# apcamargo/genomad

Hardware: NVIDIA H100
Metric: nn_classification_windows_per_s (higher is better)
Workload: dtype split operands on wgmma (conv: fp16 main pass + two e4m3 correction passes; w_v: 3 fp16 passes), fp32 accumulate; fp32-equivalent (<=1e-4 vs the fp32 oracle, measured ~1e-5)

## Files before the change

### genomad_b200/csrc/api.cu

```cuda
#include <cuda.h>
#include <cuda_runtime.h>
#include <cuda_fp16.h>

#include <algorithm>
#include <cmath>
#include <cstdio>
#include <cstring>
#include <string>
#include <vector>

#include <cub/device/device_radix_sort.cuh>
#include <cub/device/device_scan.cuh>

#include "../../include/gnm.h"
#include "common.cuh"
#include "encode.cuh"
#include "conv_t.cuh"
#include "layer1_wv.cuh"
#include "conv_ref.cuh"
#include "igloo.cuh"
#include "dense.cuh"
#include "logits_tc.cuh"
#include "wv_gather.cuh"
#include "contigs.cuh"
// ... 295 lines not shown
                                float* ent_w, int32_t* groups, int* n_groups, int32_t* band_first_group, uint32_t* frag, float* unscale,
                                int* layout) {
  if (layout) { layout[0] = kBandRows; layout[1] = kNumBands; layout[2] = kGsSlots; layout[3] = kWgGroupMax; }
  if (!patches && !w_mult && !w_summer) return 0;
  if (!patches || !w_mult || !w_summer || !n_groups) return fail("gnm_pack_patches: null argument");
  for (int i = 0; i < kPatches * kPatchLen; ++i)
    if (patches[i] < 0 || patches[i] >= kTok) return fail("gnm_pack_patches: patch index out of range");
  PatchPack pk;
  if (!pack_patches(patches, w_mult, w_summer, pk))
    return fail("gnm_pack_patches: folded patch weights w_mult * w_summer / 32 not finite: no fp16 operand split carries them");
  const int real_groups = pk.band_gstart[kNumBands];
  if (groups && *n_groups < real_groups) return fail("gnm_pack_patches: groups buffer too small");
  if (slot_of) std::memcpy(slot_of, pk.slot_of.data(), pk.slot_of.size() * sizeof(int32_t));
  if (ent_pos) std::memcpy(ent_pos, pk.ent_pos.data(), pk.ent_pos.size() * sizeof(int32_t));
  if (ent_w) std::memcpy(ent_w, pk.ent_w.data(), pk.ent_w.size() * sizeof(float));
  if (groups) for (int i = 0; i < real_groups; ++i) { groups[2 * i] = pk.groups[i].x; groups[2 * i + 1] = pk.groups[i].y; }
  *n_groups = real_groups;
  if (band_first_group) std::memcpy(band_first_group, pk.band_gstart.data(), pk.band_gstart.size() * sizeof(int32_t));
  if (frag) std::memcpy(frag, pk.frag.data(), pk.frag.size() * sizeof(uint32_t));
  if (unscale) *unscale = pk.unscale;
  return 0;
}

static void fold_bn(const gnm_bn_weights& b, std::vector<float>& sc, std::vector<float>& sh) {
  sc.resize(kHidden); sh.resize(kHidden);
  for (int i = 0; i < kHidden; ++i) {
    const float inv = b.gamma[i] * (1.0f / std::sqrt(b.moving_variance[i] + 1e-3f));
    sc[i] = inv;
    sh[i] = b.beta[i] - b.moving_mean[i] * inv;
  }
}

static void split_dense_t(const float* w, int K, std::vector<float>& thi, std::vector<float>& tlo) {
  thi.resize(static_cast<size_t>(kHidden) * K); tlo.resize(thi.size());
  for (int k = 0; k < K; ++k)
    for (int n = 0; n < kHidden; ++n)
      split_tf32(w[static_cast<size_t>(k) * kHidden + n], thi[static_cast<size_t>(n) * K + k], tlo[static_cast<size_t>(n) * K + k]);
}

extern "C" int gnm_create(int device, const gnm_weights* w, int max_batch, gnm_handle** out) {
  if (!w || !out) return fail("gnm_create: null argument");
  if (max_batch < 1 || max_batch > 32768) return fail("gnm_create: max_batch must be in [1, 32768]");
  int ndev = 0;
  if (cudaGetDeviceCount(&ndev) != cudaSuccess || ndev == 0)
    return fail("gnm_create: no CUDA device available (libgnm has no CPU fallback)");
  if (device < 0 || device >= ndev) return fail("gnm_create: bad device index");
// ... 2529 lines not shown
```

### genomad_b200/csrc/conv_t.cuh

```cuda
#pragma once
#include <cuda.h>
#include "common.cuh"

namespace gnm {

constexpr int kTileM       = 128;
constexpr int kUnitsPerWin = (kTok + 2 * kTileM - 1) / (2 * kTileM);
constexpr int kSlabRows    = 136;
constexpr int kARegion     = kSlabRows * 128;
constexpr int kA2Region    = 2 * kARegion;
constexpr int kNumRegions  = 4;
constexpr int kA2Bytes     = kNumRegions * kA2Region;
constexpr int kBStage      = 128 * 128;
constexpr int kBHalf       = kBStage / 2;
constexpr int kConvThreads = 384;
constexpr int kConvStages  = 24;
constexpr int kWvStages    = 4;
constexpr int kTWSlots     = 5;
constexpr int kEpiTile     = 512;
constexpr int kEpiStage    = 8 * 2 * kEpiTile;
constexpr int kConvTSmem   = kA2Bytes + 2 * kTWSlots * kBHalf + kEpiStage + 2048;
static_assert(kConvTSmem <= 232448, "conv_t_kernel exceeds the 227 KB of shared memory a CTA may use");

struct ConvTcParams {
  const float* bias;
  uint8_t* y_out;
  float* q_out;
  float out_scale;
  int out_fp8;
  int n_tiles;
  int experiment;
  long long* dbg;
  DeviceStatus* status;
};

template <bool kWvMode> __device__ __forceinline__ int conv_pack_stage(int q) {
  return kWvMode ? q : ((q / 6 + 2) & 3) * 6 + q % 6;
}
template <bool kWvMode> __device__ __forceinline__ constexpr int region_src(int r) {
  return kWvMode ? (r == 0 ? kOffHi16 : r == 1 ? kOffHi16 + 128 : r == 2 ? kOffLo16 : kOffLo16 + 128)
                 : (r == 0 ? kOffHi16 : r == 1 ? kOffHi16 + 128 : r == 2 ? kOffP8 : kOffP8 + 128);
}

constexpr int kConvFwd = 0, kConvWv = 1, kConvRoute = 2, kConvBwd = 3;
struct ConvAttrExt {
  uint8_t* route_out;
  const uint8_t* mask_rows;
  const float* add_rows;
  const float* s_w;
  const float* s_in;
  float* f32_out;
  float* unit_max;
};

template <int kMode>
__device__ __forceinline__ void conv_t_body(const CUtensorMap* tm_act_p, const CUtensorMap* tm_w_p, const ConvTcParams& p,
                                            const ConvAttrExt& x) {
  constexpr bool kWvMode = kMode == kConvWv || kMode == kConvRoute;
  constexpr int kStagesU = kWvMode ? kWvStages : kConvStages;
  extern __shared__ uint8_t smem_raw[];
  uint8_t* smem = reinterpret_cast<uint8_t*>((reinterpret_cast<uintptr_t>(smem_raw) + 1023) & ~uintptr_t(1023));
  uint8_t* s_a = smem;
  uint8_t* s_w = smem + kA2Bytes;
  uint8_t* s_epi = s_w + 2 * kTWSlots * kBHalf;
  uint64_t* bars = reinterpret_cast<uint64_t*>(s_epi + kEpiStage);
  uint64_t* a_full = bars;
  uint64_t* a_empty = bars + 4;
  uint64_t* w_full = bars + 8;
  uint64_t* w_empty = bars + 8 + 2 * kTWSlots;

  const int warp = __shfl_sync(0xffffffffu, static_cast<int>(threadIdx.x) >> 5, 0);
  const int wg = warp >> 2, wq = warp & 3, lane = threadIdx.x & 31;
  const int n_units = p.n_tiles;

  if (threadIdx.x == 0) {
    tma_prefetch_desc(tm_act_p);
    tma_prefetch_desc(tm_w_p);
    for (int i = 0; i < kNumRegions; ++i) { mbar_init(&a_full[i], 1); mbar_init(&a_empty[i], 8); }
    for (int i = 0; i < 2 * kTWSlots; ++i) { mbar_init(&w_full[i], 1); mbar_init(&w_empty[i], 4); }
    fence_barrier_init();
  }
  __syncthreads();

  if (wg == 0) {
    if (wq == 0 && elect_one()) {
      uint32_t wcount = 0;
      const uint64_t pol = l2_policy_evict_last();
      for (int unit = blockIdx.x; unit < n_units; unit += gridDim.x, wcount += kStagesU)
        for (int g = 0; g < 2; ++g)
          for (int q = 0; q < kStagesU; ++q) {
            const int s = g * kTWSlots + (wcount + q) % kTWSlots;
            const uint32_t wphase = ((wcount + q) / kTWSlots) & 1;
            mbar_wait(&w_empty[s], wphase ^ 1, p.status, 110 + s);
            mbar_arrive_expect_tx(&w_full[s], kBHalf);
            tma_load_2d_hint(s_w + s * kBHalf, tm_w_p, &w_full[s], 0, conv_pack_stage<kWvMode>(q) * 128 + 64 * g, pol);
          }
    } else if (wq == 1 && elect_one()) {
      int it = 0;
      const uint64_t pol = l2_policy_evict_first();
      for (int unit = blockIdx.x; unit < n_units; unit += gridDim.x, ++it) {
        const uint32_t ph = it & 1;
        const int w = unit / kUnitsPerWin;
        const int t0 = (unit - w * kUnitsPerWin) * (2 * kTileM);
#pragma unroll
        for (int k = 0; k < kNumRegions; ++k) {
          const int r = kWvMode ? (k == 0 ? 0 : k == 1 ? 2 : k == 2 ? 1 : 3) : (k + 2) & 3;
          mbar_wait(&a_empty[r], ph ^ 1, p.status, 100 + r);
          mbar_arrive_expect_tx(&a_full[r], kA2Region);
          uint8_t* dst = s_a + r * kA2Region;
          tma_load_3d_hint(dst, tm_act_p, &a_full[r], region_src<kWvMode>(r), t0 - 5, w, pol);
          tma_load_3d_hint(dst + kARegion, tm_act_p, &a_full[r], region_src<kWvMode>(r), t0 - 5 + kSlabRows, w, pol);
        }
      }
    }
  } else {
    const int g = wg - 1;
    const uint32_t a_base = smem_u32(s_a);
    const uint32_t w_base = smem_u32(s_w);
    const int ch0 = g * 64 + wq * 16 + (lane >> 2);
    const float bias0 = (kWvMode || kMode == kConvBwd) ? 0.f : p.bias[ch0], bias1 = (kWvMode || kMode == kConvBwd) ? 0.f : p.bias[ch0 + 8];
    const float oscale = p.out_scale;
    float amax = 0.f;
    int it = 0;
    long long w_a = 0, w_w = 0, t_mma = 0, t_epi = 0, tq;
    const long long t_begin = clock64();
    float d[128];
    for (int unit = blockIdx.x; unit < n_units; unit += gridDim.x, ++it) {
      const uint32_t aph = it & 1;
      const int w = unit / kUnitsPerWin;
      const int t0 = (unit - w * kUnitsPerWin) * (2 * kTileM);
      const uint32_t wc0 = static_cast<uint32_t>(it) * kStagesU;
      const long long t_unit = clock64();
      int prev_s = 0, prev_region = -1;
#pragma unroll
      for (int q = 0; q < kStagesU; ++q) {
        const int reg = kWvMode ? (q >> 1) : ((q / 6 + 2) & 3);
        const int tap = kWvMode ? 5 : (q % 6);
        const bool first_use = kWvMode ? ((q & 1) == 0) : (tap == 0);
        if (first_use) {
          tq = clock64();
          mbar_wait(&a_full[reg], aph, p.status, 210 + reg);
          if (kWvMode) mbar_wait(&a_full[2 + reg], aph, p.status, 214 + reg);
          w_a += clock64() - tq;
        }
        const uint32_t c = wc0 + q;
        const int s = g * kTWSlots + c % kTWSlots;
        const uint32_t wphase = (c / kTWSlots) & 1;
        tq = clock64();
        mbar_wait(&w_full[s], wphase, p.status, 220 + s);
        w_w += clock64() - tq;
        const uint64_t wdesc = gmma_desc_sw128(w_base + s * kBHalf);
        const uint64_t y0 = gmma_desc_sw128(a_base + reg * kA2Region + tap * 128);
        wgmma_fence();
        int rel = -1;
        if (kWvMode) {
          const uint64_t y1 = gmma_desc_sw128(a_base + (2 + reg) * kA2Region + tap * 128);
          const bool w_lo = (q & 1) != 0;
#pragma unroll
          for (int kk = 0; kk < 4; ++kk) {
            wgmma_f16_n256(d, wdesc + kk * 2, y0 + kk * 2, (q == 0 && kk == 0) ? 0u : 1u);
            if (!w_lo) wgmma_f16_n256(d, wdesc + kk * 2, y1 + kk * 2, 1u);
          }
          rel = q == 0 ? 2 : q == 1 ? 0 : q == 2 ? 3 : 1;
        } else {
          if (reg >= 2) {
#pragma unroll
            for (int kk = 0; kk < 4; ++kk) wgmma_e4m3_n256(d, wdesc + kk * 2, y0 + kk * 2, (q == 0 && kk == 0) ? 0u : 1u);
          } else {
#pragma unroll
            for (int kk = 0; kk < 4; ++kk) wgmma_f16_n256(d, wdesc + kk * 2, y0 + kk * 2, 1u);
          }
          if (tap == 5) rel = reg;
        }
        wgmma_commit();
        wgmma_wait<1>();
        if (q > 0) {
          __syncwarp();
          if (lane == 0) {
            mbar_arrive(&w_empty[prev_s]);
            if (prev_region >= 0) mbar_arrive(&a_empty[prev_region]);
          }
        }
        prev_s = s; prev_region = rel;
      }
      wgmma_wait<0>();
      __syncwarp();
      if (lane == 0) {
        mbar_arrive(&w_empty[prev_s]);
        if (prev_region >= 0) mbar_arrive(&a_empty[prev_region]);
      }
      wgmma_fence_regs(d);
      tq = clock64();
      t_mma += tq - t_unit;
      if constexpr (kMode == kConvRoute) {
        const int r0 = 2 * (lane & 3);
#pragma unroll
        for (int j = 0; j < 32; ++j) {
          float v[2];
          int ix[2];
#pragma unroll
          for (int h = 0; h < 2; ++h) {
            const float a = d[4 * j + 2 * h], b = d[4 * j + 2 * h + 1];
            v[h] = b > a ? b : a;
            ix[h] = b > a ? r0 + 1 : r0;
          }
#pragma unroll
          for (int off = 1; off <= 2; off <<= 1)
#pragma unroll
            for (int h = 0; h < 2; ++h) {
              const float pv = __shfl_xor_sync(0xffffffffu, v[h], off);
              const int pi = __shfl_xor_sync(0xffffffffu, ix[h], off);
              if (pv > v[h] || (pv == v[h] && pi < ix[h])) { v[h] = pv; ix[h] = pi; }
            }
          const int gg = (t0 >> 3) + j;
          if ((lane & 3) == 0 && gg < kPooled) {
            const size_t o = (static_cast<size_t>(w) * kPooled + gg) * kC;
            p.q_out[o + ch0] = v[0] * oscale;
            p.q_out[o + ch0 + 8] = v[1] * oscale;
            x.route_out[o + ch0] = static_cast<uint8_t>(ix[0]);
            x.route_out[o + ch0 + 8] = static_cast<uint8_t>(ix[1]);
          }
        }
      } else if (kWvMode) {
#pragma unroll
        for (int j = 0; j < 32; ++j) {
          float m0 = fmaxf(d[4 * j], d[4 * j + 1]), m1 = fmaxf(d[4 * j + 2], d[4 * j + 3]);
          m0 = fmaxf(m0, __shfl_xor_sync(0xffffffffu, m0, 1)); m1 = fmaxf(m1, __shfl_xor_sync(0xffffffffu, m1, 1));
          m0 = fmaxf(m0, __shfl_xor_sync(0xffffffffu, m0, 2)); m1 = fmaxf(m1, __shfl_xor_sync(0xffffffffu, m1, 2));
          const int gg = (t0 >> 3) + j;
          if ((lane & 3) == 0 && gg < kPooled) {
            float* qrow = p.q_out + (static_cast<size_t>(w) * kPooled + gg) * kC;
            qrow[ch0] = m0 * oscale;
            qrow[ch0 + 8] = m1 * oscale;
          }
        }
      } else if constexpr (kMode == kConvBwd) {
        const float sw = x.add_rows ? x.s_w[w] : 0.f;
        const float inv = x.s_in ? 1.f / x.s_in[w] : 1.f;
        float umax = 0.f;
#pragma unroll
        for (int j = 0; j < 32; ++j)
#pragma unroll
          for (int h = 0; h < 2; ++h)
#pragma unroll
            for (int e = 0; e < 2; ++e) {
              const int pos = t0 + 8 * j + 2 * (lane & 3) + e;
              if (pos < kTok) {
                const int ch = ch0 + 8 * h;
                const size_t row = static_cast<size_t>(w) * kTok + (kTok - 1 - pos);
                float v = d[4 * j + 2 * h + e] * oscale;
                if (x.s_in) v *= inv;
                if (x.add_rows) v = fmaf(sw, x.add_rows[row * kC + ch], v);
                const __half m = *reinterpret_cast<const __half*>(x.mask_rows + row * kRowBytes + kOffHi16 + 2 * ch);
                v = __hgt(m, __float2half(0.f)) ? v : v * kLeaky;
                x.f32_out[row * kC + ch] = v;
                umax = fmaxf(umax, fabsf(v));
              }
            }
        if (x.unit_max) {
#pragma unroll
          for (int off = 16; off > 0; off >>= 1) umax = fmaxf(umax, __shfl_xor_sync(0xffffffffu, umax, off));
          if (lane == 0) x.unit_max[static_cast<size_t>(unit) * 8 + g * 4 + wq] = umax;
        }
      } else {
        const bool store = !(p.experiment & 2);
        const uint32_t tile = smem_u32(s_epi) + (g * 4 + wq) * 2 * kEpiTile;
        const int sp = lane & 7, lp = lane >> 2;
        const uint32_t st_addr = tile + sp * 64 + (((lane >> 3) ^ (sp >> 1)) << 4);
        const uint32_t ld_addr = tile + lp * 64 + (((lane & 3) ^ (lp >> 1)) << 4);
        uint8_t* const dst = p.y_out + (static_cast<size_t>(w) * kTok + t0 + lp) * kRowBytes
                             + ((lane & 2) ? (p.out_fp8 ? kOffP8 : kOffLo16) : kOffHi16) + 2 * (g * 64 + wq * 16) + 16 * (lane & 1);
#pragma unroll
        for (int j = 0; j < 32; ++j) {
          uint32_t r[4];
#pragma unroll
          for (int h = 0; h < 2; ++h) {
            const float bias = h ? bias1 : bias0;
            const float y0 = kActScale * lrelu(fmaf(d[4 * j + 2 * h], oscale, bias));
            const float y1 = kActScale * lrelu(fmaf(d[4 * j + 2 * h + 1], oscale, bias));
            amax = fmaxf(amax, fmaxf(fabsf(y0), fabsf(y1)));
            if (p.out_fp8) {
              const __half2 hh = __floats2half2_rn(y0, y1);
              const float2 f = __half22float2(hh);
              const uint32_t e0 = pack_e4m3x2((y0 - f.x) * kLo8Scale, f.x * kHi8Scale);
              const uint32_t e1 = pack_e4m3x2((y1 - f.y) * kLo8Scale, f.y * kHi8Scale);
              r[h] = pack_h2(__low2half(hh), __high2half(hh));
              r[2 + h] = e0 | (e1 << 16);
            } else {
              __half2 hh, l;
              split2_f16(y0, y1, hh, l);
              r[h] = pack_h2(__low2half(hh), __high2half(hh));
              r[2 + h] = pack_h2(__low2half(l), __high2half(l));
            }
          }
          const uint32_t buf = (j & 1) * kEpiTile;
          stmatrix_x4_trans(st_addr + buf, r[0], r[1], r[2], r[3]);
          __syncwarp();
          const uint4 v = ld_shared_v4(ld_addr + buf);
          if (store && t0 + 8 * j + lp < kTok) *reinterpret_cast<uint4*>(dst + static_cast<size_t>(8 * j) * kRowBytes) = v;
        }
      }
      t_epi += clock64() - tq;
    }
    if constexpr (!kWvMode && kMode != kConvBwd) flag_act_overflow(p.status, amax, p.out_fp8 ? kHi8Limit : kF16Limit, p.out_fp8 ? 2 : 3);
    if (p.dbg && wq == 0 && lane == 0) {
      long long* dd = p.dbg + blockIdx.x * 8;
      if (g == 0) { dd[0] = clock64() - t_begin; dd[1] = t_mma; dd[2] = w_a; dd[3] = w_w; dd[4] = it; dd[6] = t_epi; }
      else { dd[5] = t_mma; dd[7] = t_epi; }
    }
  }
}

template <bool kWvMode>
__global__ void __launch_bounds__(kConvThreads, 1)
conv_t_kernel(const __grid_constant__ CUtensorMap tm_act, const __grid_constant__ CUtensorMap tm_w,
              const ConvTcParams p) {
  conv_t_body<kWvMode ? kConvWv : kConvFwd>(&tm_act, &tm_w, p, ConvAttrExt{});
}

template <int kMode>
__global__ void __launch_bounds__(kConvThreads, 1)
conv_t_attr_kernel(const __grid_constant__ CUtensorMap tm_act, const __grid_constant__ CUtensorMap tm_w,
                   const ConvTcParams p, const ConvAttrExt x) {
  conv_t_body<kMode>(&tm_act, &tm_w, p, x);
// ... 4 lines not shown
```

### genomad_b200/csrc/wgmma.cuh

```cuda
#pragma once
#include <stdint.h>

namespace gnm {

__device__ __forceinline__ void wgmma_fence() { asm volatile("wgmma.fence.sync.aligned;" ::: "memory"); }
__device__ __forceinline__ void wgmma_commit() { asm volatile("wgmma.commit_group.sync.aligned;" ::: "memory"); }
template <int kPending> __device__ __forceinline__ void wgmma_wait() {
  asm volatile("wgmma.wait_group.sync.aligned %0;" ::"n"(kPending) : "memory");
}
template <int kN> __device__ __forceinline__ void wgmma_fence_regs(float (&d)[kN]) {
#pragma unroll
  for (int i = 0; i < kN; ++i) asm volatile("" : "+f"(d[i])::"memory");
}

__device__ __forceinline__ uint64_t gmma_desc_sw128(uint32_t saddr) {
  uint64_t d = 0;
  d |= static_cast<uint64_t>((saddr & 0x3FFFF) >> 4);
  d |= static_cast<uint64_t>(1) << 16;
  d |= static_cast<uint64_t>(1024 >> 4) << 32;
  d |= static_cast<uint64_t>(1) << 62;
  return d;
}

#define GNM_ACC8(b) "+f"(d[b]), "+f"(d[b + 1]), "+f"(d[b + 2]), "+f"(d[b + 3]), "+f"(d[b + 4]), "+f"(d[b + 5]), "+f"(d[b + 6]), "+f"(d[b + 7])
// ... 1 lines not shown
  asm volatile("{\n.reg .pred p;\nsetp.ne.b32 p, %26, 0;\n"
               "wgmma.mma_async.sync.aligned.m64n48k16.f32.f16.f16 {%0,%1,%2,%3,%4,%5,%6,%7,%8,%9,%10,%11,%12,%13,%14,%15,%16,%17,%18,%19,%20,%21,%22,%23}, %24,%25,p,1,1,0,0;\n}"
               : GNM_ACC8(0), GNM_ACC8(8), GNM_ACC8(16)
               : "l"(da), "l"(db), "r"(accumulate));
}
__device__ __forceinline__ void wgmma_f16_n192(float (&d)[96], uint64_t da, uint64_t db, uint32_t accumulate) {
  asm volatile("{\n.reg .pred p;\nsetp.ne.b32 p, %98, 0;\n"
               "wgmma.mma_async.sync.aligned.m64n192k16.f32.f16.f16 {%0,%1,%2,%3,%4,%5,%6,%7,%8,%9,%10,%11,%12,%13,%14,%15,%16,%17,%18,%19,%20,%21,%22,%23,%24,%25,%26,%27,%28,%29,%30,%31,%32,%33,%34,%35,%36,%37,%38,%39,%40,%41,%42,%43,%44,%45,%46,%47,%48,%49,%50,%51,%52,%53,%54,%55,%56,%57,%58,%59,%60,%61,%62,%63,%64,%65,%66,%67,%68,%69,%70,%71,%72,%73,%74,%75,%76,%77,%78,%79,%80,%81,%82,%83,%84,%85,%86,%87,%88,%89,%90,%91,%92,%93,%94,%95}, %96,%97,p,1,1,0,0;\n}"
               : GNM_ACC8(0), GNM_ACC8(8), GNM_ACC8(16), GNM_ACC8(24), GNM_ACC8(32), GNM_ACC8(40), GNM_ACC8(48), GNM_ACC8(56), GNM_ACC8(64), GNM_ACC8(72), GNM_ACC8(80), GNM_ACC8(88)
               : "l"(da), "l"(db), "r"(accumulate));
}
__device__ __forceinline__ void wgmma_f16_n256(float (&d)[128], uint64_t da, uint64_t db, uint32_t accumulate) {
  asm volatile("{\n.reg .pred p;\nsetp.ne.b32 p, %130, 0;\n"
               "wgmma.mma_async.sync.aligned.m64n256k16.f32.f16.f16 {%0,%1,%2,%3,%4,%5,%6,%7,%8,%9,%10,%11,%12,%13,%14,%15,%16,%17,%18,%19,%20,%21,%22,%23,%24,%25,%26,%27,%28,%29,%30,%31,%32,%33,%34,%35,%36,%37,%38,%39,%40,%41,%42,%43,%44,%45,%46,%47,%48,%49,%50,%51,%52,%53,%54,%55,%56,%57,%58,%59,%60,%61,%62,%63,%64,%65,%66,%67,%68,%69,%70,%71,%72,%73,%74,%75,%76,%77,%78,%79,%80,%81,%82,%83,%84,%85,%86,%87,%88,%89,%90,%91,%92,%93,%94,%95,%96,%97,%98,%99,%100,%101,%102,%103,%104,%105,%106,%107,%108,%109,%110,%111,%112,%113,%114,%115,%116,%117,%118,%119,%120,%121,%122,%123,%124,%125,%126,%127}, %128,%129,p,1,1,0,0;\n}"
               : GNM_ACC8(0), GNM_ACC8(8), GNM_ACC8(16), GNM_ACC8(24), GNM_ACC8(32), GNM_ACC8(40), GNM_ACC8(48), GNM_ACC8(56), GNM_ACC8(64), GNM_ACC8(72), GNM_ACC8(80), GNM_ACC8(88), GNM_ACC8(96), GNM_ACC8(104), GNM_ACC8(112), GNM_ACC8(120)
               : "l"(da), "l"(db), "r"(accumulate));
}
__device__ __forceinline__ void wgmma_e4m3_n256(float (&d)[128], uint64_t da, uint64_t db, uint32_t accumulate) {
  asm volatile("{\n.reg .pred p;\nsetp.ne.b32 p, %130, 0;\n"
               "wgmma.mma_async.sync.aligned.m64n256k32.f32.e4m3.e4m3 {%0,%1,%2,%3,%4,%5,%6,%7,%8,%9,%10,%11,%12,%13,%14,%15,%16,%17,%18,%19,%20,%21,%22,%23,%24,%25,%26,%27,%28,%29,%30,%31,%32,%33,%34,%35,%36,%37,%38,%39,%40,%41,%42,%43,%44,%45,%46,%47,%48,%49,%50,%51,%52,%53,%54,%55,%56,%57,%58,%59,%60,%61,%62,%63,%64,%65,%66,%67,%68,%69,%70,%71,%72,%73,%74,%75,%76,%77,%78,%79,%80,%81,%82,%83,%84,%85,%86,%87,%88,%89,%90,%91,%92,%93,%94,%95,%96,%97,%98,%99,%100,%101,%102,%103,%104,%105,%106,%107,%108,%109,%110,%111,%112,%113,%114,%115,%116,%117,%118,%119,%120,%121,%122,%123,%124,%125,%126,%127}, %128,%129,p,1,1;\n}"
               : GNM_ACC8(0), GNM_ACC8(8), GNM_ACC8(16), GNM_ACC8(24), GNM_ACC8(32), GNM_ACC8(40), GNM_ACC8(48), GNM_ACC8(56), GNM_ACC8(64), GNM_ACC8(72), GNM_ACC8(80), GNM_ACC8(88), GNM_ACC8(96), GNM_ACC8(104), GNM_ACC8(112), GNM_ACC8(120)
               : "l"(da), "l"(db), "r"(accumulate));
}
__device__ __forceinline__ void wgmma_tf32_n256(float (&d)[128], uint64_t da, uint64_t db, uint32_t accumulate) {
  asm volatile("{\n.reg .pred p;\nsetp.ne.b32 p, %130, 0;\n"
               "wgmma.mma_async.sync.aligned.m64n256k8.f32.tf32.tf32 {%0,%1,%2,%3,%4,%5,%6,%7,%8,%9,%10,%11,%12,%13,%14,%15,%16,%17,%18,%19,%20,%21,%22,%23,%24,%25,%26,%27,%28,%29,%30,%31,%32,%33,%34,%35,%36,%37,%38,%39,%40,%41,%42,%43,%44,%45,%46,%47,%48,%49,%50,%51,%52,%53,%54,%55,%56,%57,%58,%59,%60,%61,%62,%63,%64,%65,%66,%67,%68,%69,%70,%71,%72,%73,%74,%75,%76,%77,%78,%79,%80,%81,%82,%83,%84,%85,%86,%87,%88,%89,%90,%91,%92,%93,%94,%95,%96,%97,%98,%99,%100,%101,%102,%103,%104,%105,%106,%107,%108,%109,%110,%111,%112,%113,%114,%115,%116,%117,%118,%119,%120,%121,%122,%123,%124,%125,%126,%127}, %128,%129,p,1,1;\n}"
               : GNM_ACC8(0), GNM_ACC8(8), GNM_ACC8(16), GNM_ACC8(24), GNM_ACC8(32), GNM_ACC8(40), GNM_ACC8(48), GNM_ACC8(56), GNM_ACC8(64), GNM_ACC8(72), GNM_ACC8(80), GNM_ACC8(88), GNM_ACC8(96), GNM_ACC8(104), GNM_ACC8(112), GNM_ACC8(120)
               : "l"(da), "l"(db), "r"(accumulate));
}
__device__ __forceinline__ void wgmma_tf32_n192(float (&d)[96], uint64_t da, uint64_t db, uint32_t accumulate) {
  asm volatile("{\n.reg .pred p;\nsetp.ne.b32 p, %98, 0;\n"
               "wgmma.mma_async.sync.aligned.m64n192k8.f32.tf32.tf32 {%0,%1,%2,%3,%4,%5,%6,%7,%8,%9,%10,%11,%12,%13,%14,%15,%16,%17,%18,%19,%20,%21,%22,%23,%24,%25,%26,%27,%28,%29,%30,%31,%32,%33,%34,%35,%36,%37,%38,%39,%40,%41,%42,%43,%44,%45,%46,%47,%48,%49,%50,%51,%52,%53,%54,%55,%56,%57,%58,%59,%60,%61,%62,%63,%64,%65,%66,%67,%68,%69,%70,%71,%72,%73,%74,%75,%76,%77,%78,%79,%80,%81,%82,%83,%84,%85,%86,%87,%88,%89,%90,%91,%92,%93,%94,%95}, %96,%97,p,1,1;\n}"
               : GNM_ACC8(0), GNM_ACC8(8), GNM_ACC8(16), GNM_ACC8(24), GNM_ACC8(32), GNM_ACC8(40), GNM_ACC8(48), GNM_ACC8(56), GNM_ACC8(64), GNM_ACC8(72), GNM_ACC8(80), GNM_ACC8(88)
               : "l"(da), "l"(db), "r"(accumulate));
}
#undef GNM_ACC8

}
```

### genomad_b200/engine.py

```python
from __future__ import annotations

import ctypes as C
import os
from pathlib import Path
from typing import Dict, List, NamedTuple, Optional, Tuple

import numpy as np

from . import weights as _weights

_PKG = Path(__file__).resolve().parent
_LIB_PATH = Path(os.environ["GENOMAD_B200_LIB"]) if os.environ.get("GENOMAD_B200_LIB") else _PKG / "libgnm.so"
_lib = None

WINDOW = 6000
TOKENS = 5997
EMBED = 512


class GnmError(RuntimeError):
    pass


class _IglooW(C.Structure):
# ... 37 lines not shown
                                     C.c_void_p, C.POINTER(C.c_int64), C.c_void_p]),
    "gnm_contig_windows_stride": (C.c_int, [C.c_void_p, C.c_void_p, C.c_void_p, C.c_int, C.c_int, C.c_void_p, C.c_void_p,
                                            C.c_int64, C.c_void_p, C.POINTER(C.c_int64), C.c_void_p]),
    "gnm_contig_windows_rc": (C.c_int, [C.c_void_p, C.c_void_p, C.c_void_p, C.c_int, C.c_int, C.c_int, C.c_void_p, C.c_void_p,
                                        C.c_int64, C.c_void_p, C.POINTER(C.c_int64), C.c_void_p]),
    "gnm_gather_windows": (C.c_int, [C.c_void_p, C.c_void_p, C.c_void_p, C.c_void_p, C.c_int, C.c_void_p, C.c_void_p]),
    "gnm_gather_windows_rc": (C.c_int, [C.c_void_p, C.c_void_p, C.c_void_p, C.c_void_p, C.c_int, C.c_void_p, C.c_void_p]),
    "gnm_forward_windows": (C.c_int, [C.c_void_p, C.c_void_p, C.c_void_p, C.c_void_p, C.c_int, C.c_void_p, C.c_void_p]),
    "gnm_forward_windows_rc": (C.c_int, [C.c_void_p, C.c_void_p, C.c_void_p, C.c_void_p, C.c_int, C.c_void_p, C.c_void_p]),
    "gnm_embed_tokens": (C.c_int, [C.c_void_p, C.c_void_p, C.c_int, C.c_void_p, C.c_void_p, C.c_void_p]),
    "gnm_embed_ascii": (C.c_int, [C.c_void_p, C.c_void_p, C.c_int, C.c_void_p, C.c_void_p, C.c_void_p]),
    "gnm_embed_windows": (C.c_int, [C.c_void_p, C.c_void_p, C.c_void_p, C.c_void_p, C.c_int, C.c_void_p, C.c_void_p, C.c_void_p]),
    "gnm_embed_windows_rc": (C.c_int, [C.c_void_p, C.c_void_p, C.c_void_p, C.c_void_p, C.c_int, C.c_void_p, C.c_void_p,
                                       C.c_void_p]),
    "gnm_embed_host": (C.c_int, [C.c_void_p, C.c_void_p, C.c_int, C.c_void_p, C.c_void_p]),
    "gnm_segment_sum_rows": (C.c_int, [C.c_void_p, C.c_void_p, C.c_void_p, C.c_int, C.c_void_p, C.c_void_p, C.c_void_p, C.c_void_p]),
    "gnm_set_option": (C.c_int, [C.c_void_p, C.c_char_p, C.c_int]),
    "gnm_get_option": (C.c_int, [C.c_void_p, C.c_char_p, C.POINTER(C.c_int)]),
    "gnm_kernel_launches": (C.c_longlong, [C.c_void_p]),
    "gnm_stage_times": (C.c_int, [C.c_void_p, C.POINTER(C.c_char_p), C.POINTER(C.c_float), C.POINTER(C.c_int)]),
    "gnm_debug_fetch": (C.c_int, [C.c_void_p, C.c_char_p, C.c_int, C.c_void_p, C.c_void_p]),
    "gnm_pack_patches": (C.c_int, [C.c_void_p, C.c_void_p, C.c_void_p, C.c_void_p, C.c_void_p, C.c_void_p, C.c_void_p,
                                   C.POINTER(C.c_int), C.c_void_p, C.c_void_p, C.POINTER(C.c_float), C.c_void_p]),
    "gnm_attr_create": (C.c_int, [C.c_void_p, C.c_int, C.POINTER(C.c_void_p)]),
    "gnm_attr_destroy": (C.c_int, [C.c_void_p]),
    "gnm_attr_bytes_per_window": (C.c_longlong, []),
    "gnm_attribute_ascii": (C.c_int, [C.c_void_p, C.c_void_p, C.c_void_p, C.c_int, C.c_int, C.c_void_p, C.c_void_p, C.c_void_p]),
    "gnm_attribute_windows": (C.c_int, [C.c_void_p, C.c_void_p, C.c_void_p, C.c_void_p, C.c_void_p, C.c_int, C.c_int, C.c_void_p,
                                        C.c_void_p, C.c_void_p]),
    "gnm_attribute_ig_ascii": (C.c_int, [C.c_void_p, C.c_void_p, C.c_void_p, C.c_int, C.c_int, C.c_int, C.c_int, C.c_void_p,
                                         C.c_void_p, C.c_void_p, C.c_void_p]),
    "gnm_attribute_ig_windows": (C.c_int, [C.c_void_p, C.c_void_p, C.c_void_p, C.c_void_p, C.c_void_p, C.c_int, C.c_int, C.c_int,
                                           C.c_int, C.c_void_p, C.c_void_p, C.c_void_p, C.c_void_p]),
    "gnm_attribute_head_ascii": (C.c_int, [C.c_void_p, C.c_void_p, C.c_void_p, C.c_void_p, C.c_int, C.c_int, C.c_void_p,
                                           C.c_void_p, C.c_void_p, C.c_void_p]),
    "gnm_attribute_head_windows": (C.c_int, [C.c_void_p, C.c_void_p, C.c_void_p, C.c_void_p, C.c_void_p, C.c_void_p, C.c_int,
                                             C.c_int, C.c_void_p, C.c_void_p, C.c_void_p, C.c_void_p]),
    "gnm_attribute_head_ig_ascii": (C.c_int, [C.c_void_p, C.c_void_p, C.c_void_p, C.c_void_p, C.c_int, C.c_int, C.c_int, C.c_int,
                                              C.c_void_p, C.c_void_p, C.c_void_p, C.c_void_p, C.c_void_p]),
    "gnm_attribute_head_ig_windows": (C.c_int, [C.c_void_p, C.c_void_p, C.c_void_p, C.c_void_p, C.c_void_p, C.c_void_p, C.c_int,
                                                C.c_int, C.c_int, C.c_int, C.c_void_p, C.c_void_p, C.c_void_p, C.c_void_p,
                                                C.c_void_p]),
    "gnm_attribute_novelty_ascii": (C.c_int, [C.c_void_p, C.c_void_p, C.c_void_p, C.c_void_p, C.c_int, C.c_void_p, C.c_void_p,
                                              C.c_void_p, C.c_void_p, C.c_void_p]),
    "gnm_attribute_novelty_windows": (C.c_int, [C.c_void_p, C.c_void_p, C.c_void_p, C.c_void_p, C.c_void_p, C.c_void_p, C.c_int,
                                                C.c_void_p, C.c_void_p, C.c_void_p, C.c_void_p, C.c_void_p]),
# ... 1691 lines not shown
```

### include/gnm.h

```cpp
#ifndef GNM_H_
#define GNM_H_

#include <stddef.h>
#include <stdint.h>

#ifdef __cplusplus
extern "C" {
#endif

#define GNM_WINDOW 6000
#define GNM_TOKENS 5997
#define GNM_CLASSES 3
#define GNM_EMBED 512

typedef struct gnm_handle gnm_handle;

typedef struct gnm_igloo_weights {
  const float*   w_mult;
  const float*   w_summer;
  const float*   w_bias;
  const float*   w_qk;
  const float*   w_v;
  const int32_t* patches;
} gnm_igloo_weights;
// ... 98 lines not shown
const char* gnm_tsv_last_error(void);
int gnm_write_window_tsv(const char* path, const char* header, const char* names, const int64_t* name_offsets, int64_t n_contigs,
                         const int32_t* win_offsets, const int64_t* starts, const int32_t* lengths, const float* probs,
                         int threads);
int gnm_write_window_tsv_cols(const char* path, const char* header, const char* names, const int64_t* name_offsets,
                              int64_t n_contigs, const int32_t* win_offsets, const int64_t* starts, const int32_t* lengths,
                              const float* probs, int n_cols, int threads);
int gnm_format_scores(const float* x, int64_t n, char* out, int64_t* out_len);


const char* gnm_tfrecord_last_error(void);
int gnm_tfrecord_write(const char* path, const uint16_t* tokens, int64_t n, int threads);
int gnm_tfrecord_read(const char* path, uint16_t* tokens, int64_t capacity, int64_t* n_records);
uint32_t gnm_crc32c(const void* data, size_t n);


int gnm_set_option(gnm_handle* h, const char* name, int value);
int gnm_get_option(gnm_handle* h, const char* name, int* value);

int gnm_pack_patches(const int32_t* patches, const float* w_mult, const float* w_summer, int32_t* slot_of, int32_t* ent_pos,
                     float* ent_w, int32_t* groups, int* n_groups, int32_t* band_first_group, uint32_t* frag, float* unscale,
                     int* layout);

long long gnm_kernel_launches(gnm_handle* h);

int gnm_stage_times(gnm_handle* h, const char** names, float* ms, int* count);

int gnm_debug_fetch(gnm_handle* h, const char* which, int n, float* d_dst, void* stream);

typedef struct gnm_attr gnm_attr;
int gnm_attr_create(gnm_handle* h, int max_batch, gnm_attr** out);
int gnm_attr_destroy(gnm_attr* a);
long long gnm_attr_bytes_per_window(void);
int gnm_attribute_ascii(gnm_handle* h, gnm_attr* a, const uint8_t* d_ascii, int n, int target, float* d_probs, float* d_attr,
                        void* stream);
int gnm_attribute_windows(gnm_handle* h, gnm_attr* a, const uint8_t* d_seq, const int64_t* d_win_start, const int32_t* d_win_len,
                          int n, int target, float* d_probs, float* d_attr, void* stream);

#define GNM_IG_BASELINE_ZERO 0
#define GNM_IG_BASELINE_N    1
int gnm_attribute_ig_ascii(gnm_handle* h, gnm_attr* a, const uint8_t* d_ascii, int n, int target, int steps, int baseline,
                           float* d_probs, float* d_logp, float* d_attr, void* stream);
int gnm_attribute_ig_windows(gnm_handle* h, gnm_attr* a, const uint8_t* d_seq, const int64_t* d_win_start,
                             const int32_t* d_win_len, int n, int target, int steps, int baseline, float* d_probs, float* d_logp,
                             float* d_attr, void* stream);

// ... 115 lines not shown
```

Before: 83470.

## Use narrower n112 wgmma for each window's tail conv unit and rotate unit order

The last 256-token unit of each window covers only about 112 real tokens, so it now runs m64n112 wgmma instructions instead of n256 and skips the padded columns. Unit indices are also permuted per window so the short units spread across CTAs instead of landing on the same ones. The MMA and epilogue code is split out into templated helpers, and an exported helper reports the unit order. The tradeoffs are larger code from two template instantiations and the risk that the epilogue still walks all 32 groups using stale accumulator values for the short tile.

```diff
diff --git a/genomad_b200/csrc/api.cu b/genomad_b200/csrc/api.cu
--- a/genomad_b200/csrc/api.cu
+++ b/genomad_b200/csrc/api.cu
@@ -341,6 +341,12 @@
   return 0;
 }
 
+extern "C" int gnm_conv_unit_order(int n_windows, int32_t* unit_of) {
+  if (n_windows < 1 || !unit_of) return fail("gnm_conv_unit_order: needs n_windows >= 1 and a unit_of array");
+  for (int i = 0; i < n_windows * kUnitsPerWin; ++i) unit_of[i] = conv_unit_of(i);
+  return 0;
+}
+
 static void fold_bn(const gnm_bn_weights& b, std::vector<float>& sc, std::vector<float>& sh) {
   sc.resize(kHidden); sh.resize(kHidden);
   for (int i = 0; i < kHidden; ++i) {
diff --git a/genomad_b200/csrc/conv_t.cuh b/genomad_b200/csrc/conv_t.cuh
--- a/genomad_b200/csrc/conv_t.cuh
+++ b/genomad_b200/csrc/conv_t.cuh
@@ -21,6 +21,20 @@
 constexpr int kEpiStage    = 8 * 2 * kEpiTile;
 constexpr int kConvTSmem   = kA2Bytes + 2 * kTWSlots * kBHalf + kEpiStage + 2048;
 static_assert(kConvTSmem <= 232448, "conv_t_kernel exceeds the 227 KB of shared memory a CTA may use");
+constexpr int kShortN      = (kTok - (kUnitsPerWin - 1) * 2 * kTileM + 7) / 8 * 8;
+static_assert(kShortN == 112 && (kUnitsPerWin - 1) * 2 * kTileM + kShortN >= kTok, "short unit must cover the window's tail");
+
+__host__ __device__ __forceinline__ int conv_unit_of(int i) {
+  const int w = i / kUnitsPerWin;
+  return w * kUnitsPerWin + (i - w * kUnitsPerWin + w) % kUnitsPerWin;
+}
+
+template <int kN, int kAcc> __device__ __forceinline__ void wgmma_f16_n(float (&d)[kAcc], uint64_t da, uint64_t db, uint32_t acc) {
+  if constexpr (kN == 256) wgmma_f16_n256(d, da, db, acc); else { static_assert(kN == 112); wgmma_f16_n112(d, da, db, acc); }
+}
+template <int kN, int kAcc> __device__ __forceinline__ void wgmma_e4m3_n(float (&d)[kAcc], uint64_t da, uint64_t db, uint32_t acc) {
+  if constexpr (kN == 256) wgmma_e4m3_n256(d, da, db, acc); else { static_assert(kN == 112); wgmma_e4m3_n112(d, da, db, acc); }
+}
 
 struct ConvTcParams {
   const float* bias;
@@ -52,6 +66,187 @@
   float* f32_out;
   float* unit_max;
 };
+
+template <bool kWvMode, int kN>
+__device__ __forceinline__ void conv_mma_unit(float (&d)[128], uint32_t a_base, uint32_t w_base, int g, uint32_t wc0, uint32_t aph,
+                                              uint64_t* a_full, uint64_t* a_empty, uint64_t* w_full, uint64_t* w_empty, int lane,
+                                              DeviceStatus* status, long long& w_a, long long& w_w) {
+  constexpr int kStagesU = kWvMode ? kWvStages : kConvStages;
+  long long tq;
+  int prev_s = 0, prev_region = -1;
+#pragma unroll
+  for (int q = 0; q < kStagesU; ++q) {
+    const int reg = kWvMode ? (q >> 1) : ((q / 6 + 2) & 3);
+    const int tap = kWvMode ? 5 : (q % 6);
+    const bool first_use = kWvMode ? ((q & 1) == 0) : (tap == 0);
+    if (first_use) {
+      tq = clock64();
+      mbar_wait(&a_full[reg], aph, status, 210 + reg);
+      if (kWvMode) mbar_wait(&a_full[2 + reg], aph, status, 214 + reg);
+      w_a += clock64() - tq;
+    }
+    const uint32_t c = wc0 + q;
+    const int s = g * kTWSlots + c % kTWSlots;
+    const uint32_t wphase = (c / kTWSlots) & 1;
+    tq = clock64();
+    mbar_wait(&w_full[s], wphase, status, 220 + s);
+    w_w += clock64() - tq;
+    const uint64_t wdesc = gmma_desc_sw128(w_base + s * kBHalf);
+    const uint64_t y0 = gmma_desc_sw128(a_base + reg * kA2Region + tap * 128);
+    wgmma_fence();
+    int rel = -1;
+    if (kWvMode) {
+      const uint64_t y1 = gmma_desc_sw128(a_base + (2 + reg) * kA2Region + tap * 128);
+      const bool w_lo = (q & 1) != 0;
+#pragma unroll
+      for (int kk = 0; kk < 4; ++kk) {
+        wgmma_f16_n<kN>(d, wdesc + kk * 2, y0 + kk * 2, (q == 0 && kk == 0) ? 0u : 1u);
+        if (!w_lo) wgmma_f16_n<kN>(d, wdesc + kk * 2, y1 + kk * 2, 1u);
+      }
+      rel = q == 0 ? 2 : q == 1 ? 0 : q == 2 ? 3 : 1;
+    } else {
+      if (reg >= 2) {
+#pragma unroll
+        for (int kk = 0; kk < 4; ++kk) wgmma_e4m3_n<kN>(d, wdesc + kk * 2, y0 + kk * 2, (q == 0 && kk == 0) ? 0u : 1u);
+      } else {
+#pragma unroll
+        for (int kk = 0; kk < 4; ++kk) wgmma_f16_n<kN>(d, wdesc + kk * 2, y0 + kk * 2, 1u);
+      }
+      if (tap == 5) rel = reg;
+    }
+    wgmma_commit();
+    wgmma_wait<1>();
+    if (q > 0) {
+      __syncwarp();
+      if (lane == 0) {
+        mbar_arrive(&w_empty[prev_s]);
+        if (prev_region >= 0) mbar_arrive(&a_empty[prev_region]);
+      }
+    }
+    prev_s = s; prev_region = rel;
+  }
+  wgmma_wait<0>();
+  __syncwarp();
+  if (lane == 0) {
+    mbar_arrive(&w_empty[prev_s]);
+    if (prev_region >= 0) mbar_arrive(&a_empty[prev_region]);
+  }
+}
+
+template <int kMode, int kGroups>
+__device__ __forceinline__ void conv_epilogue(float (&d)[128], const ConvTcParams& p, const ConvAttrExt& x, uint8_t* s_epi, int unit,
+                                              int w, int t0, int g, int wq, int lane, int ch0, float bias0, float bias1, float oscale,
+                                              float& amax) {
+  constexpr bool kWvMode = kMode == kConvWv || kMode == kConvRoute;
+  if constexpr (kMode == kConvRoute) {
+    const int r0 = 2 * (lane & 3);
+#pragma unroll
+    for (int j = 0; j < kGroups; ++j) {
+      float v[2];
+      int ix[2];
+#pragma unroll
+      for (int h = 0; h < 2; ++h) {
+        const float a = d[4 * j + 2 * h], b = d[4 * j + 2 * h + 1];
+        v[h] = b > a ? b : a;
+        ix[h] = b > a ? r0 + 1 : r0;
+      }
+#pragma unroll
+      for (int off = 1; off <= 2; off <<= 1)
+#pragma unroll
+        for (int h = 0; h < 2; ++h) {
+          const float pv = __shfl_xor_sync(0xffffffffu, v[h], off);
+          const int pi = __shfl_xor_sync(0xffffffffu, ix[h], off);
+          if (pv > v[h] || (pv == v[h] && pi < ix[h])) { v[h] = pv; ix[h] = pi; }
+        }
+      const int gg = (t0 >> 3) + j;
+      if ((lane & 3) == 0 && gg < kPooled) {
+        const size_t o = (static_cast<size_t>(w) * kPooled + gg) * kC;
+        p.q_out[o + ch0] = v[0] * oscale;
+        p.q_out[o + ch0 + 8] = v[1] * oscale;
+        x.route_out[o + ch0] = static_cast<uint8_t>(ix[0]);
+        x.route_out[o + ch0 + 8] = static_cast<uint8_t>(ix[1]);
+      }
+    }
+  } else if (kWvMode) {
+#pragma unroll
+    for (int j = 0; j < kGroups; ++j) {
+      float m0 = fmaxf(d[4 * j], d[4 * j + 1]), m1 = fmaxf(d[4 * j + 2], d[4 * j + 3]);
+      m0 = fmaxf(m0, __shfl_xor_sync(0xffffffffu, m0, 1)); m1 = fmaxf(m1, __shfl_xor_sync(0xffffffffu, m1, 1));
+      m0 = fmaxf(m0, __shfl_xor_sync(0xffffffffu, m0, 2)); m1 = fmaxf(m1, __shfl_xor_sync(0xffffffffu, m1, 2));
+      const int gg = (t0 >> 3) + j;
+      if ((lane & 3) == 0 && gg < kPooled) {
+        float* qrow = p.q_out + (static_cast<size_t>(w) * kPooled + gg) * kC;
+        qrow[ch0] = m0 * oscale;
+        qrow[ch0 + 8] = m1 * oscale;
+      }
+    }
+  } else if constexpr (kMode == kConvBwd) {
+    const float sw = x.add_rows ? x.s_w[w] : 0.f;
+    const float inv = x.s_in ? 1.f / x.s_in[w] : 1.f;
+    float umax = 0.f;
+#pragma unroll
+    for (int j = 0; j < kGroups; ++j)
+#pragma unroll
+      for (int h = 0; h < 2; ++h)
+#pragma unroll
+        for (int e = 0; e < 2; ++e) {
+          const int pos = t0 + 8 * j + 2 * (lane & 3) + e;
+          if (pos < kTok) {
+            const int ch = ch0 + 8 * h;
+            const size_t row = static_cast<size_t>(w) * kTok + (kTok - 1 - pos);
+            float v = d[4 * j + 2 * h + e] * oscale;
+            if (x.s_in) v *= inv;
+            if (x.add_rows) v = fmaf(sw, x.add_rows[row * kC + ch], v);
+            const __half m = *reinterpret_cast<const __half*>(x.mask_rows + row * kRowBytes + kOffHi16 + 2 * ch);
+            v = __hgt(m, __float2half(0.f)) ? v : v * kLeaky;
+            x.f32_out[row * kC + ch] = v;
+            umax = fmaxf(umax, fabsf(v));
+          }
+        }
+    if (x.unit_max) {
+#pragma unroll
+      for (int off = 16; off > 0; off >>= 1) umax = fmaxf(umax, __shfl_xor_sync(0xffffffffu, umax, off));
+      if (lane == 0) x.unit_max[static_cast<size_t>(unit) * 8 + g * 4 + wq] = umax;
+    }
+  } else {
+    const bool store = !(p.experiment & 2);
+    const uint32_t tile = smem_u32(s_epi) + (g * 4 + wq) * 2 * kEpiTile;
+    const int sp = lane & 7, lp = lane >> 2;
+    const uint32_t st_addr = tile + sp * 64 + (((lane >> 3) ^ (sp >> 1)) << 4);
+    const uint32_t ld_addr = tile + lp * 64 + (((lane & 3) ^ (lp >> 1)) << 4);
+    uint8_t* const dst = p.y_out + (static_cast<size_t>(w) * kTok + t0 + lp) * kRowBytes
+                         + ((lane & 2) ? (p.out_fp8 ? kOffP8 : kOffLo16) : kOffHi16) + 2 * (g * 64 + wq * 16) + 16 * (lane & 1);
+#pragma unroll
+    for (int j = 0; j < kGroups; ++j) {
+      uint32_t r[4];
+#pragma unroll
+      for (int h = 0; h < 2; ++h) {
+        const float bias = h ? bias1 : bias0;
+        const float y0 = kActScale * lrelu(fmaf(d[4 * j + 2 * h], oscale, bias));
+        const float y1 = kActScale * lrelu(fmaf(d[4 * j + 2 * h + 1], oscale, bias));
+        amax = fmaxf(amax, fmaxf(fabsf(y0), fabsf(y1)));
+        if (p.out_fp8) {
+          const __half2 hh = __floats2half2_rn(y0, y1);
+          const float2 f = __half22float2(hh);
+          const uint32_t e0 = pack_e4m3x2((y0 - f.x) * kLo8Scale, f.x * kHi8Scale);
+          const uint32_t e1 = pack_e4m3x2((y1 - f.y) * kLo8Scale, f.y * kHi8Scale);
+          r[h] = pack_h2(__low2half(hh), __high2half(hh));
+          r[2 + h] = e0 | (e1 << 16);
+        } else {
+          __half2 hh, l;
+          split2_f16(y0, y1, hh, l);
+          r[h] = pack_h2(__low2half(hh), __high2half(hh));
+          r[2 + h] = pack_h2(__low2half(l), __high2half(l));
+        }
+      }
+      const uint32_t buf = (j & 1) * kEpiTile;
+      stmatrix_x4_trans(st_addr + buf, r[0], r[1], r[2], r[3]);
+      __syncwarp();
+      const uint4 v = ld_shared_v4(ld_addr + buf);
+      if (store && t0 + 8 * j + lp < kTok) *reinterpret_cast<uint4*>(dst + static_cast<size_t>(8 * j) * kRowBytes) = v;
+    }
+  }
+}
 
 template <int kMode>
 __device__ __forceinline__ void conv_t_body(const CUtensorMap* tm_act_p, const CUtensorMap* tm_w_p, const ConvTcParams& p,
@@ -86,7 +281,7 @@
     if (wq == 0 && elect_one()) {
       uint32_t wcount = 0;
       const uint64_t pol = l2_policy_evict_last();
-      for (int unit = blockIdx.x; unit < n_units; unit += gridDim.x, wcount += kStagesU)
+      for (int i = blockIdx.x; i < n_units; i += gridDim.x, wcount += kStagesU)
         for (int g = 0; g < 2; ++g)
           for (int q = 0; q < kStagesU; ++q) {
             const int s = g * kTWSlots + (wcount + q) % kTWSlots;
@@ -98,8 +293,9 @@
     } else if (wq == 1 && elect_one()) {
       int it = 0;
       const uint64_t pol = l2_policy_evict_first();
-      for (int unit = blockIdx.x; unit < n_units; unit += gridDim.x, ++it) {
+      for (int i = blockIdx.x; i < n_units; i += gridDim.x, ++it) {
         const uint32_t ph = it & 1;
+        const int unit = conv_unit_of(i);
         const int w = unit / kUnitsPerWin;
         const int t0 = (unit - w * kUnitsPerWin) * (2 * kTileM);
 #pragma unroll
@@ -125,181 +321,24 @@
     long long w_a = 0, w_w = 0, t_mma = 0, t_epi = 0, tq;
     const long long t_begin = clock64();
     float d[128];
-    for (int unit = blockIdx.x; unit < n_units; unit += gridDim.x, ++it) {
+#pragma unroll
+    for (int k = 0; k < 128; ++k) d[k] = 0.f;
+    for (int i = blockIdx.x; i < n_units; i += gridDim.x, ++it) {
       const uint32_t aph = it & 1;
+      const int unit = conv_unit_of(i);
       const int w = unit / kUnitsPerWin;
       const int t0 = (unit - w * kUnitsPerWin) * (2 * kTileM);
+      const bool short_unit = unit - w * kUnitsPerWin == kUnitsPerWin - 1;
       const uint32_t wc0 = static_cast<uint32_t>(it) * kStagesU;
       const long long t_unit = clock64();
-      int prev_s = 0, prev_region = -1;
-#pragma unroll
-      for (int q = 0; q < kStagesU; ++q) {
-        const int reg = kWvMode ? (q >> 1) : ((q / 6 + 2) & 3);
-        const int tap = kWvMode ? 5 : (q % 6);
-        const bool first_use = kWvMode ? ((q & 1) == 0) : (tap == 0);
-        if (first_use) {
-          tq = clock64();
-          mbar_wait(&a_full[reg], aph, p.status, 210 + reg);
-          if (kWvMode) mbar_wait(&a_full[2 + reg], aph, p.status, 214 + reg);
-          w_a += clock64() - tq;
-        }
-        const uint32_t c = wc0 + q;
-        const int s = g * kTWSlots + c % kTWSlots;
-        const uint32_t wphase = (c / kTWSlots) & 1;
-        tq = clock64();
-        mbar_wait(&w_full[s], wphase, p.status, 220 + s);
-        w_w += clock64() - tq;
-        const uint64_t wdesc = gmma_desc_sw128(w_base + s * kBHalf);
-        const uint64_t y0 = gmma_desc_sw128(a_base + reg * kA2Region + tap * 128);
-        wgmma_fence();
-        int rel = -1;
-        if (kWvMode) {
-          const uint64_t y1 = gmma_desc_sw128(a_base + (2 + reg) * kA2Region + tap * 128);
-          const bool w_lo = (q & 1) != 0;
-#pragma unroll
-          for (int kk = 0; kk < 4; ++kk) {
-            wgmma_f16_n256(d, wdesc + kk * 2, y0 + kk * 2, (q == 0 && kk == 0) ? 0u : 1u);
-            if (!w_lo) wgmma_f16_n256(d, wdesc + kk * 2, y1 + kk * 2, 1u);
-          }
-          rel = q == 0 ? 2 : q == 1 ? 0 : q == 2 ? 3 : 1;
-        } else {
-          if (reg >= 2) {
-#pragma unroll
-            for (int kk = 0; kk < 4; ++kk) wgmma_e4m3_n256(d, wdesc + kk * 2, y0 + kk * 2, (q == 0 && kk == 0) ? 0u : 1u);
-          } else {
-#pragma unroll
-            for (int kk = 0; kk < 4; ++kk) wgmma_f16_n256(d, wdesc + kk * 2, y0 + kk * 2, 1u);
-          }
-          if (tap == 5) rel = reg;
-        }
-        wgmma_commit();
-        wgmma_wait<1>();
-        if (q > 0) {
-          __syncwarp();
-          if (lane == 0) {
-            mbar_arrive(&w_empty[prev_s]);
-            if (prev_region >= 0) mbar_arrive(&a_empty[prev_region]);
-          }
-        }
-        prev_s = s; prev_region = rel;
-      }
-      wgmma_wait<0>();
-      __syncwarp();
-      if (lane == 0) {
-        mbar_arrive(&w_empty[prev_s]);
-        if (prev_region >= 0) mbar_arrive(&a_empty[prev_region]);
-      }
+      if (short_unit)
+        conv_mma_unit<kWvMode, kShortN>(d, a_base, w_base, g, wc0, aph, a_full, a_empty, w_full, w_empty, lane, p.status, w_a, w_w);
+      else
+        conv_mma_unit<kWvMode, 2 * kTileM>(d, a_base, w_base, g, wc0, aph, a_full, a_empty, w_full, w_empty, lane, p.status, w_a, w_w);
       wgmma_fence_regs(d);
       tq = clock64();
       t_mma += tq - t_unit;
-      if constexpr (kMode == kConvRoute) {
-        const int r0 = 2 * (lane & 3);
-#pragma unroll
-        for (int j = 0; j < 32; ++j) {
-          float v[2];
-          int ix[2];
-#pragma unroll
-          for (int h = 0; h < 2; ++h) {
-            const float a = d[4 * j + 2 * h], b = d[4 * j + 2 * h + 1];
-            v[h] = b > a ? b : a;
-            ix[h] = b > a ? r0 + 1 : r0;
-          }
-#pragma unroll
-          for (int off = 1; off <= 2; off <<= 1)
-#pragma unroll
-            for (int h = 0; h < 2; ++h) {
-              const float pv = __shfl_xor_sync(0xffffffffu, v[h], off);
-              const int pi = __shfl_xor_sync(0xffffffffu, ix[h], off);
-              if (pv > v[h] || (pv == v[h] && pi < ix[h])) { v[h] = pv; ix[h] = pi; }
-            }
-          const int gg = (t0 >> 3) + j;
-          if ((lane & 3) == 0 && gg < kPooled) {
-            const size_t o = (static_cast<size_t>(w) * kPooled + gg) * kC;
-            p.q_out[o + ch0] = v[0] * oscale;
-            p.q_out[o + ch0 + 8] = v[1] * oscale;
-            x.route_out[o + ch0] = static_cast<uint8_t>(ix[0]);
-            x.route_out[o + ch0 + 8] = static_cast<uint8_t>(ix[1]);
-          }
-        }
-      } else if (kWvMode) {
-#pragma unroll
-        for (int j = 0; j < 32; ++j) {
-          float m0 = fmaxf(d[4 * j], d[4 * j + 1]), m1 = fmaxf(d[4 * j + 2], d[4 * j + 3]);
-          m0 = fmaxf(m0, __shfl_xor_sync(0xffffffffu, m0, 1)); m1 = fmaxf(m1, __shfl_xor_sync(0xffffffffu, m1, 1));
-          m0 = fmaxf(m0, __shfl_xor_sync(0xffffffffu, m0, 2)); m1 = fmaxf(m1, __shfl_xor_sync(0xffffffffu, m1, 2));
-          const int gg = (t0 >> 3) + j;
-          if ((lane & 3) == 0 && gg < kPooled) {
-            float* qrow = p.q_out + (static_cast<size_t>(w) * kPooled + gg) * kC;
-            qrow[ch0] = m0 * oscale;
-            qrow[ch0 + 8] = m1 * oscale;
-          }
-        }
-      } else if constexpr (kMode == kConvBwd) {
-        const float sw = x.add_rows ? x.s_w[w] : 0.f;
-        const float inv = x.s_in ? 1.f / x.s_in[w] : 1.f;
-        float umax = 0.f;
-#pragma unroll
-        for (int j = 0; j < 32; ++j)
-#pragma unroll
-          for (int h = 0; h < 2; ++h)
-#pragma unroll
-            for (int e = 0; e < 2; ++e) {
-              const int pos = t0 + 8 * j + 2 * (lane & 3) + e;
-              if (pos < kTok) {
-                const int ch = ch0 + 8 * h;
-                const size_t row = static_cast<size_t>(w) * kTok + (kTok - 1 - pos);
-                float v = d[4 * j + 2 * h + e] * oscale;
-                if (x.s_in) v *= inv;
-                if (x.add_rows) v = fmaf(sw, x.add_rows[row * kC + ch], v);
-                const __half m = *reinterpret_cast<const __half*>(x.mask_rows + row * kRowBytes + kOffHi16 + 2 * ch);
-                v = __hgt(m, __float2half(0.f)) ? v : v * kLeaky;
-                x.f32_out[row * kC + ch] = v;
-                umax = fmaxf(umax, fabsf(v));
-              }
-            }
-        if (x.unit_max) {
-#pragma unroll
-          for (int off = 16; off > 0; off >>= 1) umax = fmaxf(umax, __shfl_xor_sync(0xffffffffu, umax, off));
-          if (lane == 0) x.unit_max[static_cast<size_t>(unit) * 8 + g * 4 + wq] = umax;
-        }
-      } else {
-        const bool store = !(p.experiment & 2);
-        const uint32_t tile = smem_u32(s_epi) + (g * 4 + wq) * 2 * kEpiTile;
-        const int sp = lane & 7, lp = lane >> 2;
-        const uint32_t st_addr = tile + sp * 64 + (((lane >> 3) ^ (sp >> 1)) << 4);
-        const uint32_t ld_addr = tile + lp * 64 + (((lane & 3) ^ (lp >> 1)) << 4);
-        uint8_t* const dst = p.y_out + (static_cast<size_t>(w) * kTok + t0 + lp) * kRowBytes
-                             + ((lane & 2) ? (p.out_fp8 ? kOffP8 : kOffLo16) : kOffHi16) + 2 * (g * 64 + wq * 16) + 16 * (lane & 1);
-#pragma unroll
-        for (int j = 0; j < 32; ++j) {
-          uint32_t r[4];
-#pragma unroll
-          for (int h = 0; h < 2; ++h) {
-            const float bias = h ? bias1 : bias0;
-            const float y0 = kActScale * lrelu(fmaf(d[4 * j + 2 * h], oscale, bias));
-            const float y1 = kActScale * lrelu(fmaf(d[4 * j + 2 * h + 1], oscale, bias));
-            amax = fmaxf(amax, fmaxf(fabsf(y0), fabsf(y1)));
-            if (p.out_fp8) {
-              const __half2 hh = __floats2half2_rn(y0, y1);
-              const float2 f = __half22float2(hh);
-              const uint32_t e0 = pack_e4m3x2((y0 - f.x) * kLo8Scale, f.x * kHi8Scale);
-              const uint32_t e1 = pack_e4m3x2((y1 - f.y) * kLo8Scale, f.y * kHi8Scale);
-              r[h] = pack_h2(__low2half(hh), __high2half(hh));
-              r[2 + h] = e0 | (e1 << 16);
-            } else {
-              __half2 hh, l;
-              split2_f16(y0, y1, hh, l);
-              r[h] = pack_h2(__low2half(hh), __high2half(hh));
-              r[2 + h] = pack_h2(__low2half(l), __high2half(l));
-            }
-          }
-          const uint32_t buf = (j & 1) * kEpiTile;
-          stmatrix_x4_trans(st_addr + buf, r[0], r[1], r[2], r[3]);
-          __syncwarp();
-          const uint4 v = ld_shared_v4(ld_addr + buf);
-          if (store && t0 + 8 * j + lp < kTok) *reinterpret_cast<uint4*>(dst + static_cast<size_t>(8 * j) * kRowBytes) = v;
-        }
-      }
+      conv_epilogue<kMode, 2 * kTileM / 8>(d, p, x, s_epi, unit, w, t0, g, wq, lane, ch0, bias0, bias1, oscale, amax);
       t_epi += clock64() - tq;
     }
     if constexpr (!kWvMode && kMode != kConvBwd) flag_act_overflow(p.status, amax, p.out_fp8 ? kHi8Limit : kF16Limit, p.out_fp8 ? 2 : 3);
diff --git a/genomad_b200/csrc/wgmma.cuh b/genomad_b200/csrc/wgmma.cuh
--- a/genomad_b200/csrc/wgmma.cuh
+++ b/genomad_b200/csrc/wgmma.cuh
@@ -47,6 +47,20 @@
                : GNM_ACC8(0), GNM_ACC8(8), GNM_ACC8(16), GNM_ACC8(24), GNM_ACC8(32), GNM_ACC8(40), GNM_ACC8(48), GNM_ACC8(56), GNM_ACC8(64), GNM_ACC8(72), GNM_ACC8(80), GNM_ACC8(88), GNM_ACC8(96), GNM_ACC8(104), GNM_ACC8(112), GNM_ACC8(120)
                : "l"(da), "l"(db), "r"(accumulate));
 }
+template <int kN> __device__ __forceinline__ void wgmma_f16_n112(float (&d)[kN], uint64_t da, uint64_t db, uint32_t accumulate) {
+  static_assert(kN >= 56, "m64n112 needs 56 accumulator registers");
+  asm volatile("{\n.reg .pred p;\nsetp.ne.b32 p, %58, 0;\n"
+               "wgmma.mma_async.sync.aligned.m64n112k16.f32.f16.f16 {%0,%1,%2,%3,%4,%5,%6,%7,%8,%9,%10,%11,%12,%13,%14,%15,%16,%17,%18,%19,%20,%21,%22,%23,%24,%25,%26,%27,%28,%29,%30,%31,%32,%33,%34,%35,%36,%37,%38,%39,%40,%41,%42,%43,%44,%45,%46,%47,%48,%49,%50,%51,%52,%53,%54,%55}, %56,%57,p,1,1,0,0;\n}"
+               : GNM_ACC8(0), GNM_ACC8(8), GNM_ACC8(16), GNM_ACC8(24), GNM_ACC8(32), GNM_ACC8(40), GNM_ACC8(48)
+               : "l"(da), "l"(db), "r"(accumulate));
+}
+template <int kN> __device__ __forceinline__ void wgmma_e4m3_n112(float (&d)[kN], uint64_t da, uint64_t db, uint32_t accumulate) {
+  static_assert(kN >= 56, "m64n112 needs 56 accumulator registers");
+  asm volatile("{\n.reg .pred p;\nsetp.ne.b32 p, %58, 0;\n"
+               "wgmma.mma_async.sync.aligned.m64n112k32.f32.e4m3.e4m3 {%0,%1,%2,%3,%4,%5,%6,%7,%8,%9,%10,%11,%12,%13,%14,%15,%16,%17,%18,%19,%20,%21,%22,%23,%24,%25,%26,%27,%28,%29,%30,%31,%32,%33,%34,%35,%36,%37,%38,%39,%40,%41,%42,%43,%44,%45,%46,%47,%48,%49,%50,%51,%52,%53,%54,%55}, %56,%57,p,1,1;\n}"
+               : GNM_ACC8(0), GNM_ACC8(8), GNM_ACC8(16), GNM_ACC8(24), GNM_ACC8(32), GNM_ACC8(40), GNM_ACC8(48)
+               : "l"(da), "l"(db), "r"(accumulate));
+}
 __device__ __forceinline__ void wgmma_tf32_n256(float (&d)[128], uint64_t da, uint64_t db, uint32_t accumulate) {
   asm volatile("{\n.reg .pred p;\nsetp.ne.b32 p, %130, 0;\n"
                "wgmma.mma_async.sync.aligned.m64n256k8.f32.tf32.tf32 {%0,%1,%2,%3,%4,%5,%6,%7,%8,%9,%10,%11,%12,%13,%14,%15,%16,%17,%18,%19,%20,%21,%22,%23,%24,%25,%26,%27,%28,%29,%30,%31,%32,%33,%34,%35,%36,%37,%38,%39,%40,%41,%42,%43,%44,%45,%46,%47,%48,%49,%50,%51,%52,%53,%54,%55,%56,%57,%58,%59,%60,%61,%62,%63,%64,%65,%66,%67,%68,%69,%70,%71,%72,%73,%74,%75,%76,%77,%78,%79,%80,%81,%82,%83,%84,%85,%86,%87,%88,%89,%90,%91,%92,%93,%94,%95,%96,%97,%98,%99,%100,%101,%102,%103,%104,%105,%106,%107,%108,%109,%110,%111,%112,%113,%114,%115,%116,%117,%118,%119,%120,%121,%122,%123,%124,%125,%126,%127}, %128,%129,p,1,1;\n}"
diff --git a/genomad_b200/engine.py b/genomad_b200/engine.py
--- a/genomad_b200/engine.py
+++ b/genomad_b200/engine.py
@@ -83,6 +83,7 @@
     "gnm_debug_fetch": (C.c_int, [C.c_void_p, C.c_char_p, C.c_int, C.c_void_p, C.c_void_p]),
     "gnm_pack_patches": (C.c_int, [C.c_void_p, C.c_void_p, C.c_void_p, C.c_void_p, C.c_void_p, C.c_void_p, C.c_void_p,
                                    C.POINTER(C.c_int), C.c_void_p, C.c_void_p, C.POINTER(C.c_float), C.c_void_p]),
+    "gnm_conv_unit_order": (C.c_int, [C.c_int, C.c_void_p]),
     "gnm_attr_create": (C.c_int, [C.c_void_p, C.c_int, C.POINTER(C.c_void_p)]),
     "gnm_attr_destroy": (C.c_int, [C.c_void_p]),
     "gnm_attr_bytes_per_window": (C.c_longlong, []),
diff --git a/include/gnm.h b/include/gnm.h
--- a/include/gnm.h
+++ b/include/gnm.h
@@ -144,6 +144,8 @@
                      float* ent_w, int32_t* groups, int* n_groups, int32_t* band_first_group, uint32_t* frag, float* unscale,
                      int* layout);
 
+int gnm_conv_unit_order(int n_windows, int32_t* unit_of);
+
 long long gnm_kernel_launches(gnm_handle* h);
 
 int gnm_stage_times(gnm_handle* h, const char** names, float* ms, int* count);
```

New measurement: 75330, median of 6. 9.8% lower.
